# pghysels/STRUMPACK

Measured on AMD Instinct MI355X. Metric: hss_compress_ulv_factor_solve_gflops, higher is better.
Workload: dtype f64

## Files before the change

include/hssk.h:

```cpp
#ifndef HSSK_H
#define HSSK_H

#ifdef __cplusplus
extern "C" {
#endif

typedef struct hssk_ctx hssk_ctx;

int hssk_ctx_create(hssk_ctx** ctx, int device);
void hssk_ctx_destroy(hssk_ctx* ctx);
void* hssk_ctx_stream(hssk_ctx* ctx);
int hssk_sync(hssk_ctx* ctx);
const char* hssk_last_error(void);
typedef struct hssk_plan hssk_plan;
int hssk_plan_begin(hssk_ctx* ctx, hssk_plan** plan);
int hssk_plan_end(hssk_ctx* ctx);
int hssk_plan_replay(hssk_ctx* ctx, hssk_plan* plan);
void hssk_plan_destroy(hssk_plan* plan);
int hssk_plan_size(const hssk_plan* plan);

void* hssk_malloc(long long bytes);
void hssk_free(void* dptr);
long long hssk_device_total_bytes(void);
int hssk_memcpy_h2d(hssk_ctx* ctx, void* dst, const void* src, long long bytes);
int hssk_memcpy_d2h(hssk_ctx* ctx, void* dst, const void* src, long long bytes);
int hssk_upload_async(hssk_ctx* ctx, void* dst, const void* src, long long bytes);
int hssk_memcpy_d2d(hssk_ctx* ctx, void* dst, const void* src, long long bytes);
int hssk_memcpy2d_h2d(hssk_ctx* ctx, void* dst, long long dpitch, const void* src, long long spitch,
                      long long width, long long height);
int hssk_memcpy2d_d2h(hssk_ctx* ctx, void* dst, long long dpitch, const void* src, long long spitch,
                      long long width, long long height);
int hssk_memset_zero(hssk_ctx* ctx, void* dst, long long bytes);
// ... 299 lines not shown
                    double atol, int max_rank, const hssk_elem_src* src, int* res);
int hssk_tree_rcap_max(void);

typedef struct hssk_qr_desc {
  double* A;
  int lda, rows, cols;
  double* Q;
  int ldq, nq;
  double* rdiag;
  double* work;
  int stair;
  double stop_rel, stop_abs;
  int r_only;
} hssk_qr_desc;
int hssk_qr_vbatched(hssk_ctx* ctx, const hssk_qr_desc* descs, int count);
typedef struct hssk_tpqr_desc {
  double* R1;
  int ld1;
  const double* R2;
  int ld2, m;
} hssk_tpqr_desc;
int hssk_tpqr_vbatched(hssk_ctx* ctx, const hssk_tpqr_desc* descs, int count);
int hssk_formq_vbatched(hssk_ctx* ctx, const hssk_qr_desc* descs, int count);

typedef struct hssk_trsm_desc {
  const double* T;
  double* B;
  int n, nrhs, ldt, ldb;
  int lower, transT, unit;
  const double* Tinv;
} hssk_trsm_desc;
int hssk_trsm_vbatched(hssk_ctx* ctx, const hssk_trsm_desc* descs, int count);
typedef struct hssk_lu_desc {
  double* A;
  int n, lda;
  int* piv;
  int* info;
} hssk_lu_desc;
int hssk_getrf_vbatched(hssk_ctx* ctx, const hssk_lu_desc* descs, int count);
typedef struct hssk_lusolve_desc {
  const double* LU;
  const int* piv;
  double* B;
  int n, nrhs, lda, ldb;
} hssk_lusolve_desc;
int hssk_getrs_vbatched(hssk_ctx* ctx, const hssk_lusolve_desc* descs, int count);
// ... 154 lines not shown
```

strumpack_amd/csrc/hip/hssk_rt.h:

```cpp
#pragma once
#include <hip/hip_runtime.h>

#include <cstdio>
#include <stdexcept>
#include <string>

#define HSSK_CHECK(call)                                                                      \
  do {                                                                                        \
    hipError_t e_ = (call);                                                                   \
    if (e_ != hipSuccess)                                                                     \
      throw std::runtime_error(std::string("HIP error: ") + hipGetErrorString(e_) + " at " +  \
                               __FILE__ + ":" + std::to_string(__LINE__));                    \
  } while (0)

namespace hssk_rt {
typedef hipStream_t stream_t;
typedef hipEvent_t event_t;
inline void* dev_malloc(size_t bytes) { void* p = nullptr; if (bytes) HSSK_CHECK(hipMalloc(&p, bytes)); return p; }
inline void dev_free(void* p) { if (p) (void)hipFree(p); }
inline bool pinned_is_device_visible() { return true; }
inline void* pinned_malloc(size_t bytes) { void* p = nullptr; if (bytes) HSSK_CHECK(hipHostMalloc(&p, bytes, hipHostMallocDefault)); return p; }
inline void pinned_free(void* p) { if (p) (void)hipHostFree(p); }
inline void h2d(void* d, const void* h, size_t bytes, stream_t s) { if (bytes) HSSK_CHECK(hipMemcpyAsync(d, h, bytes, hipMemcpyHostToDevice, s)); }
inline void d2h(void* h, const void* d, size_t bytes, stream_t s) { if (bytes) HSSK_CHECK(hipMemcpyAsync(h, d, bytes, hipMemcpyDeviceToHost, s)); }
inline void d2d(void* d, const void* s_, size_t bytes, stream_t s) { if (bytes) HSSK_CHECK(hipMemcpyAsync(d, s_, bytes, hipMemcpyDeviceToDevice, s)); }
inline void h2d_2d(void* d, size_t dpitch, const void* h, size_t hpitch, size_t width, size_t height, stream_t s) {
  if (width && height) HSSK_CHECK(hipMemcpy2DAsync(d, dpitch, h, hpitch, width, height, hipMemcpyHostToDevice, s));
}
inline void d2h_2d(void* h, size_t hpitch, const void* d, size_t dpitch, size_t width, size_t height, stream_t s) {
  if (width && height) HSSK_CHECK(hipMemcpy2DAsync(h, hpitch, d, dpitch, width, height, hipMemcpyDeviceToHost, s));
}
inline void memset_async(void* d, int v, size_t bytes, stream_t s) { if (bytes) HSSK_CHECK(hipMemsetAsync(d, v, bytes, s)); }
inline void sync(stream_t s) { HSSK_CHECK(hipStreamSynchronize(s)); }
inline void check_launch() { HSSK_CHECK(hipGetLastError()); }
template <typename K> inline void allow_dynamic_lds(K kernel, size_t bytes) {
  HSSK_CHECK(hipFuncSetAttribute(reinterpret_cast<const void*>(kernel), hipFuncAttributeMaxDynamicSharedMemorySize, (int)bytes));
}
inline size_t max_lds_per_workgroup() {
  int dev = 0, n = 0;
  if (hipGetDevice(&dev) != hipSuccess) { (void)hipGetLastError(); return 65536; }
  if (hipDeviceGetAttribute(&n, hipDeviceAttributeSharedMemPerBlockOptin, dev) != hipSuccess || n <= 0) {
    (void)hipGetLastError();
    if (hipDeviceGetAttribute(&n, hipDeviceAttributeMaxSharedMemoryPerBlock, dev) != hipSuccess) { (void)hipGetLastError(); return 65536; }
  }
  return n > 0 ? (size_t)n : 65536;
}
inline stream_t stream_create() { stream_t s; HSSK_CHECK(hipStreamCreateWithFlags(&s, hipStreamNonBlocking)); return s; }
inline void stream_destroy(stream_t s) { (void)hipStreamDestroy(s); }
inline event_t event_create() { event_t e; HSSK_CHECK(hipEventCreate(&e)); return e; }
inline void event_destroy(event_t e) { (void)hipEventDestroy(e); }
inline void event_record(event_t e, stream_t s) { HSSK_CHECK(hipEventRecord(e, s)); }
inline float event_elapsed_ms(event_t a, event_t b) { float ms = 0; HSSK_CHECK(hipEventSynchronize(b)); HSSK_CHECK(hipEventElapsedTime(&ms, a, b)); return ms; }
inline void stream_wait_event(stream_t s, event_t e) { HSSK_CHECK(hipStreamWaitEvent(s, e, 0)); }
inline void event_sync(event_t e) { HSSK_CHECK(hipEventSynchronize(e)); }
inline bool is_pinned_host_pointer(const void* p) {
  hipPointerAttribute_t a;
  if (hipPointerGetAttributes(&a, p) != hipSuccess) { (void)hipGetLastError(); return false; }
  return a.type == hipMemoryTypeHost;
}
inline int cu_count() {
  int dev = 0, n = 0;
  if (hipGetDevice(&dev) != hipSuccess || hipDeviceGetAttribute(&n, hipDeviceAttributeMultiprocessorCount, dev) != hipSuccess) { (void)hipGetLastError(); return 256; }
  return n > 0 ? n : 256;
}
inline int coresident_workgroups() { return cu_count(); }
inline size_t device_total_bytes() {
  size_t fr = 0, tot = 0;
  if (hipMemGetInfo(&fr, &tot) != hipSuccess) { (void)hipGetLastError(); return 0; }
  return tot;
}
inline int device_count() { int n = 0; if (hipGetDeviceCount(&n) != hipSuccess) return 0; return n; }
inline void set_device(int d) { HSSK_CHECK(hipSetDevice(d)); }
inline bool is_device_pointer(const void* p) {
  hipPointerAttribute_t a;
  if (hipPointerGetAttributes(&a, p) != hipSuccess) { (void)hipGetLastError(); return false; }
  return a.type == hipMemoryTypeDevice;
}
}
```

strumpack_amd/csrc/host/hss_engine.cpp:

```cpp
#include "hss_engine_internal.hpp"

namespace strumpack {
namespace HSS {

void CommSpec::apply(EngineOptions& e) const {
  e.world = world; e.rank = rank; e.comm_user = user;
  e.allgather = nullptr; e.allgather_stream = nullptr; e.allreduce_stream = nullptr; e.reduce_scatter_stream = nullptr;
  if (world <= 1) return;
  if (native) {
    e.allgather_stream = comm::rccl_allgather_hook;
    e.allreduce_stream = comm::rccl_allreduce_hook;
    e.reduce_scatter_stream = comm::rccl_reduce_scatter_hook;
  } else {
    e.allgather = allgather;
  }
}

DeviceHSS::DeviceHSS(int n, const EngineOptions& opts, const structured::ClusterTree* tree) : n_(n), o_(opts) {
  ck(hssk_ctx_create(&ctx_, o_.device));
  persist_.reset(new Arena(size_t(64) << 20));
  work_.reset(new Arena(size_t(256) << 20));
  fact_.reset(new Arena(size_t(64) << 20));
  tmp_.reset(new Arena(size_t(64) << 20));
  comm_arena_.reset(new Arena(size_t(64) << 20));
  plan_arena_.reset(new Arena(size_t(64) << 20));
  schur_.reset(new Arena(size_t(64) << 20));
  build_tree(tree);
  setup_ownership();
}

DeviceHSS::~DeviceHSS() {
  if (fctx_) hssk_sync(fctx_);
  if (ctx_) hssk_sync(ctx_);
  drop_plans();
  plan_arena_.reset();
  persist_.reset();
  work_.reset();
  fact_.reset();
  tmp_.reset();
  comm_arena_.reset();
  schur_.reset();
  if (fctx_) hssk_ctx_destroy(fctx_);
  hssk_ctx_destroy(ctx_);
}

void DeviceHSS::build_tree(const structured::ClusterTree* tree) {
  nodes_.clear();
  std::function<int(int, int, int, int, const structured::ClusterTree*)> rec =
      [&](int lo, int m, int lvl, int parent, const structured::ClusterTree* t) -> int {
    int id = (int)nodes_.size();
    nodes_.emplace_back();
    nodes_[id].lo = lo; nodes_[id].m = m; nodes_[id].lvl = lvl; nodes_[id].parent = parent;
    bool split = t ? !t->c.empty() : (m > o_.leaf_size);
    if (split) {
      int m0 = t ? t->c[0].size : m / 2;
      int c0 = rec(lo, m0, lvl + 1, id, t ? &t->c[0] : nullptr);
      int c1 = rec(lo + m0, m - m0, lvl + 1, id, t ? &t->c[1] : nullptr);
      nodes_[id].c0 = c0; nodes_[id].c1 = c1;
      nodes_[id].height = 1 + std::max(nodes_[c0].height, nodes_[c1].height);
    }
    return id;
  };
  if (tree && tree->size != n_) throw std::invalid_argument("cluster tree size does not match the matrix dimension");
  rec(0, n_, 0, -1, tree);
  int H = nodes_[0].height, Dp = 0;
// ... 56 lines not shown
```

strumpack_amd/csrc/host/hss_engine.hpp:

```cpp
#pragma once
#include <functional>
#include <iosfwd>
#include <map>
#include <tuple>
#include <memory>
#include <mutex>
#include <string>
#include <vector>

#include "ClusterTree.hpp"
#include "hssk.h"

namespace strumpack {
namespace HSS {

struct EngineOptions {
  double rel_tol = 1e-2, abs_tol = 1e-8;
  int leaf_size = 512, max_rank = 50000, d0 = 128, dd = 64, p = 10;
  int algorithm = 1;
  int random_engine = 0;
  int random_dist = 0;
  int sketch = 0, sjlt_algo = 0, nnz0 = 4, nnz = 4;
  bool user_random = false;
  bool factor_ahead = false;
// ... 247 lines not shown
  std::unique_ptr<Arena> comm_arena_;
  std::unique_ptr<Arena> persist_, work_, fact_, tmp_;
  double *Rt_ = nullptr, *Srt_ = nullptr, *Sct_ = nullptr;
  double *Srt0_ = nullptr, *Sct0_ = nullptr;
  int dcap_ = 0;
  int f32_route_ = 0;
  int attempt_ = 0;
  double* cut_buf_ = nullptr;
  int* cut_idx_ = nullptr;
  size_t cut_buf_cap_ = 0, cut_idx_cap_ = 0;
  int cut_gen_ = -1;
  const int* sj_pat_ = nullptr;
  int sj_nnz_ = 0;
  long long cols_per_rank_ = 0;
  int* d_ranks_ = nullptr;
  struct FactorRun {
    bool active = false, ahead = false, partial = false;
    int sr = 0;
    hssk_ctx* cx = nullptr;
    std::vector<double*> Dh, Vh, Vd;
    std::vector<hssk_trtri_desc> ti;
    std::vector<char> is_cut;
    size_t done = 0;
  } frun_;
  hssk_ctx* fctx_ = nullptr;
  void factor_begin(int sr, bool partial, hssk_ctx* cx);
  void factor_prep(const std::vector<int>& ids);
  void factor_level(const std::vector<int>& ids);
  void factor_ahead_level(size_t h);
  void factor_cancel();
  bool factored_ = false, partial_factored_ = false, schur_ready_ = false;
  void invalidate_factors() { factor_cancel(); factored_ = partial_factored_ = schur_ready_ = false; sub_factored_ = -1; }
  int sub_factored_ = -1;
  std::unique_ptr<Arena> schur_;
  void ensure_dev_tree();
  const hssk_tree_node* dev_tree_ = nullptr;
  int ex_rmax_ = 1, ex_depth_ = 1;
  double *sTheta_ = nullptr, *sPhi_ = nullptr, *sDUB01_ = nullptr, *sVtDUB01_ = nullptr, *sW_ = nullptr;
  PhaseStats stats_;
  std::shared_ptr<HostRng> rng_;
};

}
}
```

strumpack_amd/csrc/host/hss_factor.cpp:

```cpp
#include "hss_engine_internal.hpp"
#include <cstdio>

namespace strumpack {
namespace HSS {

void DeviceHSS::factor() { factor_sub(0, false); }

void DeviceHSS::partial_factor() {
  OpGuard op_guard(op_mu_);
  if (nodes_[0].leaf()) return;
  if (o_.world != 1) throw std::logic_error("partial_factor: needs a single-process matrix");
  factor_sub(nodes_[0].c0, true);
}

void DeviceHSS::factor_begin(int sr, bool partial, hssk_ctx* cx) {
  drop_plans();
  fact_->reset();
  stats_.f_ulv = 0;
  for (auto& nd : nodes_) nd.Qt = nd.Rlq = nd.W1 = nd.Vt0 = nd.Dt = nd.Vt1 = nd.LU = nd.WQ = nd.Tinv = nd.TinvU = nd.Vt0T = nd.Gc = nullptr, nd.piv = nullptr;
  chain_built_ = false;
  if (chain_arena_) chain_arena_->reset();
  const size_t nn = nodes_.size();
  frun_ = FactorRun();
  frun_.active = true;
  frun_.sr = sr; frun_.partial = partial; frun_.cx = cx;
  frun_.Dh.assign(nn, nullptr); frun_.Vh.assign(nn, nullptr); frun_.Vd.assign(nn, nullptr);
  frun_.is_cut.assign(nn, 0);
  if (dist_subtree_) for (int c : cut_nodes_) frun_.is_cut[c] = 1;
}

void DeviceHSS::factor_prep(const std::vector<int>& ids) {
  FactorRun& f = frun_;
  std::vector<hssk_basis_desc> bd;
  for (int id : ids) {
    const Node& nd = nodes_[id];
    if (id == f.sr && !f.partial) continue;
    f.Vh[id] = fact_->dbl((size_t)std::max(nd.mU, 1) * std::max(nd.rV, 1));
    if (!nd.rV) continue;
    double* out = f.Vh[id];
    if (!nd.leaf()) out = f.Vd[id] = fact_->dbl((size_t)nd.mV * nd.rV);
    bd.push_back(hssk_basis_desc{nd.XV, nd.permV, out, nd.mV, nd.rV, nd.rV, nd.mV});
  }
  if (!bd.empty()) ck(hssk_basis_dense(f.cx, bd.data(), (int)bd.size()));
}

void DeviceHSS::factor_level(const std::vector<int>& ids) {
  if (ids.empty()) return;
  FactorRun& f = frun_;
  hssk_ctx* cx = f.cx;
  const int sr = f.sr;
  const bool partial = f.partial;
  std::vector<double*>&Dh = f.Dh, &Vh = f.Vh, &Vd = f.Vd;
  auto dt_slot = [&](int id, int r, int& ld) -> double* {
    const Node& nd = nodes_[id];
    if (nd.parent < 0 || f.is_cut[id]) { ld = std::max(r, 1); return fact_->dbl((size_t)ld * ld); }
    const Node& pa = nodes_[nd.parent];
    const int mu = nodes_[pa.c0].rU + nodes_[pa.c1].rU;
    ld = std::max(mu, 1);
    if (!Dh[nd.parent]) Dh[nd.parent] = fact_->dbl((size_t)ld * ld);
    const int off = id == pa.c0 ? 0 : nodes_[pa.c0].rU;
    return Dh[nd.parent] + off + (size_t)off * ld;
  };
  static const bool no_node = [] { const char* e = std::getenv("STRUMPACK_AMD_NO_ULV_NODE"); return e && e[0] == '1'; }();
  bool fused = !no_node;
  for (int id : ids) {
    const Node& nd = nodes_[id];
// ... 40 lines not shown
      stats_.f_ulv += 2.0 * nd.rV * ((double)a.rU * a.rV + (double)b.rU * b.rV);
    }
  }
  auto node_desc = [&](int id) {
    const Node& nd = nodes_[id];
    const Node &a = nodes_[nd.c0], &b = nodes_[nd.c1];
    hssk_ulvnode_desc d{};
    d.B01 = nd.B01; d.B10 = nd.B10; d.Vt1a = a.Vt1; d.Vt1b = b.Vt1;
    d.ra = a.rU; d.rb = b.rU; d.rva = a.rV; d.rvb = b.rV;
    d.m = a.rU + b.rU;
    d.Dh = Dh[id];
    const bool vh = (id != sr || partial) && nd.rV > 0;
    d.Vd = vh ? Vd[id] : nullptr;
    d.Vh = vh ? Vh[id] : nullptr;
    d.rv = vh ? nd.rV : 0;
    return d;
  };
  if (!cp.empty()) ck(hssk_gather_cols(cx, cp.data(), (int)cp.size()));
  g0.insert(g0.end(), g1.begin(), g1.end());
  if (!g0.empty()) ck(hssk_gemm_vbatched(cx, g0.data(), (int)g0.size()));
  std::vector<hssk_elem_desc> ge;
  std::vector<hssk_ulvsplit_desc> us;
  std::vector<hssk_gemm_desc> g2, g3;
  std::vector<hssk_qr_desc> qr;
  std::vector<hssk_lu_desc> lu;
  for (int id : ids) {
    Node& nd = nodes_[id];
    if (id == sr) {
      const int mu = nd.leaf() ? nd.m : nodes_[nd.c0].rU + nodes_[nd.c1].rU;
      nd.LU = Dh[id];
      if (partial) nd.Vt0 = Vh[id];
      nd.piv = (int*)fact_->alloc(sizeof(int) * (std::max(mu, 1) + 1));
      if (mu) lu.push_back(hssk_lu_desc{nd.LU, mu, mu, nd.piv, nd.piv + mu});
      if (mu && mu <= 256) {
        const size_t nblk = (size_t)(mu + 63) / 64;
        nd.Tinv = fact_->dbl(nblk * 4096);
        nd.TinvU = fact_->dbl(nblk * 4096);
        f.ti.push_back(hssk_trtri_desc{nd.LU, nd.Tinv, mu, mu, 2});
        f.ti.push_back(hssk_trtri_desc{nd.LU, nd.TinvU, mu, mu, 1});
      }
      stats_.f_ulv += 2.0 / 3.0 * mu * (double)mu * mu;
      if (fused) un.push_back(node_desc(id));
      continue;
    }
    const int m = nd.mU, r = nd.rU, rv = nd.rV;
    if (m > r) {
// ... 10 lines not shown
        d.W1 = nd.W1; d.Rlq = nd.Rlq; d.Qt = nd.Qt; d.tau = fact_->dbl((size_t)2 * m);
        d.Vt1 = nd.Vt1; d.Dt = nd.Dt; d.ldt = ldt;
        if (rv) { nd.Vt0T = fact_->dbl((size_t)rv * (m - r)); d.Vt0T = nd.Vt0T; }
        if (r) { nd.WQ = fact_->dbl((size_t)r * (m - r)); d.WQ = nd.WQ; }
        un.push_back(d);
        nd.Tinv = fact_->dbl((size_t)((m - r + 63) / 64) * 4096);
        f.ti.push_back(hssk_trtri_desc{nd.Rlq, nd.Tinv, m - r, m, 0});
        const double k = m - r;
        stats_.f_ulv += 2.0 * k * r * m + (2.0 * m * k * k - 2.0 / 3.0 * k * k * k) + (4.0 * m * m * k - 2.0 * m * k * k) / 1.0 * 0.5 + 2.0 * m * m * rv + 2.0 * r * (double)r * m;
        continue;
      }
      if (m <= 256) {
        us.push_back(hssk_ulvsplit_desc{Dh[id], m, m, r, nd.permU, nd.XU, std::max(r, 1), nd.W1, std::max(r, 1), nd.Rlq, m});
      } else {
        if (r) ge.push_back(hssk_elem_desc{Dh[id], m, nd.permU, nullptr, 0, 0, nd.W1, r, m, r, 0});
        ge.push_back(hssk_elem_desc{Dh[id], m, nd.permU + r, nullptr, 0, 0, nd.Rlq, m - r, m, m, 1});
        if (r) g2.push_back(hssk_gemm_desc{nd.W1, nd.XU, nd.Rlq, m, m - r, r, r, r, m, 1, 0, -1.0, 1.0});
      }
      double* wk = fact_->dbl((size_t)2 * m);
      qr.push_back(hssk_qr_desc{nd.Rlq, m, m, m - r, nd.Qt, m, m, nullptr, wk});
      if (rv) {
        nd.Vt0T = fact_->dbl((size_t)rv * (m - r));
        g3.push_back(hssk_gemm_desc{Vh[id], nd.Qt, nd.Vt0T, rv, m - r, m, m, m, rv, 1, 0, 1.0, 0.0});
        if (r) g3.push_back(hssk_gemm_desc{nd.Qt + (size_t)(m - r) * m, Vh[id], nd.Vt1, r, rv, m, m, m, r, 1, 0, 1.0, 0.0});
      }
      if (r) g3.push_back(hssk_gemm_desc{nd.W1, nd.Qt + (size_t)(m - r) * m, nd.Dt, r, r, m, r, m, ldt, 0, 0, 1.0, 0.0});
      if (r) {
        nd.WQ = fact_->dbl((size_t)r * (m - r));
        g3.push_back(hssk_gemm_desc{nd.W1, nd.Qt, nd.WQ, r, m - r, m, r, m, r, 0, 0, 1.0, 0.0});
      }
      if (m <= 256) {
        nd.Tinv = fact_->dbl((size_t)((m - r + 63) / 64) * 4096);
        f.ti.push_back(hssk_trtri_desc{nd.Rlq, nd.Tinv, m - r, m, 0});
      }
      const double k = m - r;
      stats_.f_ulv += 2.0 * k * r * m + (2.0 * m * k * k - 2.0 / 3.0 * k * k * k) + (4.0 * m * m * k - 2.0 * m * k * k) / 1.0 * 0.5 + 2.0 * m * m * rv + 2.0 * r * (double)r * m;
    } else {
      int ldt = 1;
      nd.Dt = dt_slot(id, m, ldt);
      nd.Vt1 = Vh[id];
      if (m) ge.push_back(hssk_elem_desc{Dh[id], m, nd.permU, nullptr, 0, 0, nd.Dt, m, m, ldt, 0});
    }
  }
  if (!un.empty()) ck(hssk_ulv_node_vbatched(cx, un.data(), (int)un.size()));
  if (!us.empty()) ck(hssk_ulv_split(cx, us.data(), (int)us.size()));
  if (!ge.empty()) ck(hssk_gather_elems(cx, ge.data(), (int)ge.size()));
  if (!g2.empty()) ck(hssk_gemm_vbatched(cx, g2.data(), (int)g2.size()));
  if (!qr.empty()) ck(hssk_qr_vbatched(cx, qr.data(), (int)qr.size()));
  if (!g3.empty()) ck(hssk_gemm_vbatched(cx, g3.data(), (int)g3.size()));
  if (!lu.empty()) ck(hssk_getrf_vbatched(cx, lu.data(), (int)lu.size()));
}

void DeviceHSS::factor_ahead_level(size_t h) {
  if (!o_.factor_ahead || o_.algorithm != 1) return;
  if (o_.world > 1 && !dist_subtree_) return;
  if (!frun_.active) {
    if (h != 0) return;
    if (!fctx_) ck(hssk_ctx_create(&fctx_, o_.device));
    factor_begin(0, false, fctx_);
    frun_.ahead = true;
  }
  if (!frun_.ahead || h >= own_by_height_.size()) return;
  while (frun_.done <= h) {
    const std::vector<int>& ids = own_by_height_[frun_.done];
    for (int id : ids) {
      const Node& nd = nodes_[id];
      if (!nd.compressed()) return;
      if (nd.parent >= 0 && !frun_.is_cut[id]) {
        const Node& pa = nodes_[nd.parent];
        if (!nodes_[pa.c0].compressed() || !nodes_[pa.c1].compressed()) return;
      }
    }
    ck(hssk_stream_wait(fctx_, ctx_));
    factor_prep(ids);
    factor_level(ids);
    if (!frun_.ti.empty()) { ck(hssk_trtri_diag_vbatched(fctx_, frun_.ti.data(), (int)frun_.ti.size())); frun_.ti.clear(); }
    frun_.done++;
  }
}

void DeviceHSS::factor_cancel() {
  if (frun_.active && frun_.ahead && fctx_) hssk_sync(fctx_);
  frun_ = FactorRun();
}

void DeviceHSS::factor_sub(int sr, bool partial) {
  OpGuard op_guard(op_mu_);
  ensure_ready("factor");
  double t0 = now();
  std::vector<std::vector<int>> sub_h;
  if (sr != 0) sub_h = sublists(own_by_height_, sr);
  const std::vector<std::vector<int>>& levels = sr ? sub_h : own_by_height_;
  const bool resume = sr == 0 && !partial && frun_.active && frun_.ahead;
  if (resume) {
    ck(hssk_sync(fctx_));
    ck(hssk_sync(ctx_));
    frun_.cx = ctx_;
  } else {
    static const bool trace_host = [] { const char* e = std::getenv("STRUMPACK_AMD_TRACE_HOST"); return e && e[0] == '1'; }();
    const double th0 = now();
    factor_cancel();
    ck(hssk_sync(ctx_));
    const double th1 = now();
    factor_begin(sr, partial, ctx_);
    const double th2 = now();
// ... 3 lines not shown
      factor_prep(levels[0]);
      const double tp1 = now();
      factor_level(levels[0]);
      frun_.done = 1;
      if (trace_host) std::fprintf(stderr, "# host: factor: prep of the lowest level %.1f us, its launches %.1f us; since the end of compress() %.1f us\n", (tp1 - tp0) * 1e6, (now() - tp1) * 1e6, (tp0 - stats_.t_mark) * 1e6);
    }
    std::vector<int> all;
    for (size_t h = 1; h < levels.size(); h++) all.insert(all.end(), levels[h].begin(), levels[h].end());
    if (dist_subtree_) for (auto& ids : top_by_height_) all.insert(all.end(), ids.begin(), ids.end());
    factor_prep(all);
  }
  for (size_t h = frun_.done; h < levels.size(); h++) {
    if (resume) factor_prep(levels[h]);
    factor_level(levels[h]);
  }
  if (dist_subtree_) {
    exchange_cut_factor();
    for (auto& ids : top_by_height_) {
      if (resume) factor_prep(ids);
      factor_level(ids);
    }
  }
  if (!frun_.ti.empty()) ck(hssk_trtri_diag_vbatched(ctx_, frun_.ti.data(), (int)frun_.ti.size()));
  ck(hssk_sync(ctx_));
  frun_ = FactorRun();
  factored_ = sr == 0;
  sub_factored_ = (sr != 0 && !partial) ? sr : -1;
  partial_factored_ = partial;
  schur_ready_ = false;
  stats_.t_factor = now() - t0;
}

double DeviceHSS::logabsdet() {
  OpGuard op_guard(op_mu_);
  ensure_ready("logabsdet");
  if (o_.world != 1) throw std::logic_error("logabsdet: needs a single-process matrix");
  if (partial_factored_) throw std::logic_error("logabsdet: the factors come from partial_factor() (the (1,1) block is not eliminated)");
  if (!factored_) throw std::logic_error("logabsdet: factor() has not been called (or shift() invalidated the factors)");
  std::vector<hssk_logdet_desc> d;
  for (size_t id = 0; id < nodes_.size(); id++) {
    const Node& nd = nodes_[id];
    if (id == 0) {
      const int mu = nd.leaf() ? nd.m : nodes_[nd.c0].rU + nodes_[nd.c1].rU;
      if (mu) d.push_back(hssk_logdet_desc{nd.LU, mu, mu});
    } else if (nd.mU > nd.rU) {
      d.push_back(hssk_logdet_desc{nd.Rlq, nd.mU - nd.rU, nd.mU});
// ... 16 lines not shown
```

strumpack_amd/csrc/kernels/hssk_ctx.hip:

```cpp
#include "hssk_internal.h"

#include <cstdlib>
#include <unistd.h>

#include <atomic>
#include <condition_variable>
#include <functional>
#include <mutex>
#include <thread>
#include <vector>

static thread_local std::string g_err;
static std::mutex g_pool_mu;
static std::vector<hssk_ctx*> g_pool;
void hssk_set_error(const std::string& msg) { g_err = msg; }

thread_local std::vector<std::function<void()>>* hssk_rec::sink = nullptr;

struct hssk_uploader {
  static constexpr int SLOTS = 4;
  static constexpr size_t CHUNK = size_t(256) << 20;
  hssk_rt::stream_t copy{};
  hssk_rt::event_t ev_copy{}, ev_compute{};
  hssk_rt::event_t ev_mark[2];
// ... 172 lines not shown
int hssk_compute_fence(hssk_ctx* c) {
  HSSK_API_BEGIN
  hssk_uploader* u = uploader(c);
  hssk_rt::event_record(u->ev_compute, c->stream);
  hssk_rt::stream_wait_event(u->copy, u->ev_compute);
  HSSK_API_END
}
int hssk_compute_mark(hssk_ctx* c, int slot) {
  HSSK_API_BEGIN
  hssk_uploader* u = uploader(c);
  hssk_rt::event_record(u->ev_mark[slot & 1], c->stream);
  u->marked[slot & 1] = true;
  HSSK_API_END
}
int hssk_copy_wait(hssk_ctx* c, int slot) {
  HSSK_API_BEGIN
  hssk_uploader* u = uploader(c);
  if (u->marked[slot & 1]) hssk_rt::stream_wait_event(u->copy, u->ev_mark[slot & 1]);
  HSSK_API_END
}

const char* hssk_last_error(void) { return g_err.c_str(); }

int hssk_ctx_create(hssk_ctx** out, int device) {
  HSSK_API_BEGIN
  if (hssk_rt::device_count() <= device)
    throw std::runtime_error("hssk_ctx_create: no HIP device " + std::to_string(device) +
                             " (this library has no CPU fallback)");
  hssk_rt::set_device(device);
  {
    std::lock_guard<std::mutex> g(g_pool_mu);
    for (size_t i = 0; i < g_pool.size(); i++)
      if (g_pool[i]->device == device) {
        *out = g_pool[i];
        g_pool.erase(g_pool.begin() + i);
        return 0;
      }
  }
  hssk_ctx* c = new hssk_ctx;
  c->device = device;
  c->stream = hssk_rt::stream_create();
  c->ring_bytes = size_t(64) << 20;
  c->h_ring = (char*)hssk_rt::pinned_malloc(c->ring_bytes);
  c->zero_copy_bytes = hssk_rt::pinned_is_device_visible() ? 65536 : 0;
  if (const char* e = std::getenv("HSSK_ZERO_COPY_BYTES")) c->zero_copy_bytes = (size_t)std::atoll(e);
  c->d_ring = (char*)hssk_rt::dev_malloc(c->ring_bytes);
  c->ev0 = hssk_rt::event_create();
  c->ev1 = hssk_rt::event_create();
  c->ev_sync = hssk_rt::event_create();
  *out = c;
  HSSK_API_END
}

void hssk_ctx_destroy(hssk_ctx* c) {
  if (!c) return;
  try { hssk_rt::sync(c->stream); } catch (...) {}
  {
    std::lock_guard<std::mutex> g(g_pool_mu);
    if (g_pool.size() < 8) {
      if (c->uploader) c->uploader->release_slots();
      c->ring_off = 0;
      c->dgemm_timed = false;
      if (c->on_side) { c->stream = c->main_saved; c->on_side = false; }
      for (int i = 0; i < 8; i++) {
        for (auto& p : c->watch[i]) { c->watch_free.push_back(p.first); c->watch_free.push_back(p.second); }
        c->watch[i].clear();
        c->watch_open[i] = false;
      }
      c->recording = nullptr;
      c->require_mma = false;
      c->knn_filtered = 0;
      g_pool.push_back(c);
      return;
    }
// ... 268 lines not shown
```

strumpack_amd/csrc/kernels/hssk_internal.h:

```cpp
#pragma once
#include <functional>
#include <vector>
#include <algorithm>
#include <utility>
#include <cstring>
#include <stdexcept>
#include <string>

#include "hssk.h"
#include "hssk_rt.h"

namespace hssk_rec {
extern thread_local std::vector<std::function<void()>>* sink;
}

struct hssk_plan {
  std::vector<std::function<void()>> launches;
  struct Block { char* dev; char* shadow; size_t size; };
  std::vector<Block> blocks;
  size_t off = 0;
  char* alloc(size_t bytes, char** shadow) {
    const size_t need = (bytes + 255) & ~size_t(255);
    if (blocks.empty() || off + need > blocks.back().size) {
      const size_t sz = std::max<size_t>(need, size_t(1) << 20);
      blocks.push_back(Block{(char*)hssk_rt::dev_malloc(sz), (char*)hssk_rt::pinned_malloc(sz), sz});
      off = 0;
    }
    char* p = blocks.back().dev + off;
    *shadow = blocks.back().shadow + off;
    off += need;
    return p;
  }
  ~hssk_plan() { for (auto& b : blocks) { hssk_rt::dev_free(b.dev); hssk_rt::pinned_free(b.shadow); } }
};

struct hssk_uploader;
struct hssk_ctx {
  int device = 0;
  hssk_rt::stream_t stream{};
  char* h_ring = nullptr;
  char* d_ring = nullptr;
  size_t ring_bytes = 0, ring_off = 0;
  size_t zero_copy_bytes = 0;
  hssk_rt::event_t ev0{}, ev1{};
  hssk_rt::event_t ev_sync{};
  hssk_rt::stream_t side{}, main_saved{};
  hssk_rt::event_t ev_fork{}, ev_join{};
  bool on_side = false, side_made = false;
  bool require_mma = false;
  bool dgemm_timed = false;
  double dgemm_timed_flops = 0.;
  struct TimedBracket { hssk_rt::event_t a, b; double flops; };
  std::vector<TimedBracket> dgemm_deferred;
  long long dgemm_trace_wgs = 0;
  long long* d_clk = nullptr;
  double* d_scratch = nullptr;
  struct hssk_uploader* uploader = nullptr;
  int* d_sweep_flags = nullptr;
  int* h_sweep_err = nullptr;
  std::vector<std::pair<hssk_rt::event_t, hssk_rt::event_t>> watch[8];
  std::vector<hssk_rt::event_t> watch_free;
// ... 111 lines not shown
```

strumpack_amd/csrc/kernels/hssk_qr.hip:

```cpp
#include "hssk_backsub.h"
#include "hssk_device.h"
#include "hssk_internal.h"
#include "hssk_qr_reg.h"

#include <algorithm>
#include <cstdlib>
#include <vector>

namespace {

constexpr int QR_THREADS = 512;
constexpr int QR_WAVES = QR_THREADS / 64;

__global__ __launch_bounds__(QR_THREADS) void qr_kernel(const hssk_qr_desc* __restrict__ descs, int qonly) {
  HSSK_SHARED double s_tau;
  const hssk_qr_desc p = descs[blockIdx.x];
  const int tid = threadIdx.x, lane = tid & 63, wave = tid >> 6;
  const int rows = p.rows, cols = p.cols, ld = p.lda;
  double* __restrict__ A = p.A;
  double* taus = p.work;
  const int kmax = rows < cols ? rows : cols;
  double rmax = 0., rmin = 0.;

  for (int k = 0; k < (qonly ? 0 : kmax); k++) {
// ... 150 lines not shown
        hssk_row_sum_n(dot);
#pragma unroll
        for (int c = kc; c < CT; c++) {
          const int col = grp + NC * c;
          if (col > k && col < m) {
            const double tc = st[col];
            const double f = (dot[c] + tc) * tau;
#pragma unroll
            for (int r = 0; r < RC(kc); r++) a[c][r] -= f * vr[r];
            if (l16 == 0) hssk_gstore(R1, (size_t)k + (size_t)col * p.ld1, tc - f);
          }
        }
      }
      if (tid < m) s_t[((k + 1) & 1) * NC * CT + tid] = trow;
    }
  }
}
#undef RC

template <int RT, int CT, int NW>
void launch_qr_reg(hssk_ctx* ctx, const hssk_qr_desc* dd, int count) {
  HSSK_LAUNCH((qr_reg_kernel<RT, CT, NW>), dim3((unsigned)count), dim3(NW * 64), 0, ctx->stream, dd);
}
template <int RT, int CT, int NW>
void launch_formq_reg(hssk_ctx* ctx, const hssk_qr_desc* dd, const hssk_qr_desc* descs, int count) {
  std::vector<QBlock> blocks;
  for (int i = 0; i < count; i++)
    for (int b = 0; b * 4 * NW * CT < descs[i].nq; b++) blocks.push_back(QBlock{i, b});
  if (blocks.empty()) return;
  auto* dw = (const QBlock*)ctx->stage(blocks.data(), sizeof(QBlock) * blocks.size());
  HSSK_LAUNCH((formq_reg_kernel<RT, CT, NW>), dim3((unsigned)blocks.size()), dim3(NW * 64), 0, ctx->stream, dd, dw);
}
void formq_reg(hssk_ctx* ctx, const hssk_qr_desc* dd, const hssk_qr_desc* descs, int count, int rmax) {
  if (rmax <= 64) launch_formq_reg<4, 2, 8>(ctx, dd, descs, count);
  else if (rmax <= 128) launch_formq_reg<8, 4, 8>(ctx, dd, descs, count);
  else if (rmax <= 208) launch_formq_reg<13, 4, 8>(ctx, dd, descs, count);
  else launch_formq_reg<16, 4, 8>(ctx, dd, descs, count);
}

constexpr int QB = 32;
constexpr int QB_MAXROWS = 512;

struct QPanel {
  const double* A;
  const double* tau;
  double* Vc;
  double* VT;
  double* rd_panel;
  double* rdiag;
  int lda, rows, nb, ldv, first;
};

template <int MAXR, int NT>
__global__ __launch_bounds__(NT) void larft_kernel(const QPanel* __restrict__ descs) {
  constexpr int PARTS = NT >= 1024 ? 2 : 1;
  constexpr int LDV = MAXR + 1;
  constexpr int LR = HSSK_BACKSUB_LD;
  HSSK_SHARED double s_V[QB * LDV];
  HSSK_SHARED double s_G[QB * LR];
  HSSK_SHARED double s_rd[64];
// ... 504 lines not shown
    if (!fused) continue;
    for (int i = 0; i < count; i++) {
      const hssk_qr_desc& d = descs[i];
      const int kmax = std::min(d.rows, d.cols);
      if (jg >= kmax || d.nq <= jg) continue;
      WyDesc w{};
      for (int q = std::min(pmax, g0 + GP) - 1; q >= g0; q--) {
        const int jq = q * QB;
        if (jq >= kmax || d.nq <= jq) continue;
        const double* Vq = ws + offV[i] + jq + (size_t)jq * d.rows;
        w.pr[w.np++] = WyPair{Vq + (size_t)d.rows * kmax, Vq, jq - jg, std::min(QB, kmax - jq), d.rows - jq, 0};
      }
      w.C = d.Q + jg + (size_t)jg * d.ldq; w.ldv = d.rows; w.ldc = d.ldq; w.rr = d.rows - jg; w.nc = d.nq - jg;
      wy.push_back(w);
    }
    if (!wy_apply(ctx, wy)) throw std::runtime_error("hssk_qr: fused block reflector refused a block it had accepted");
  }
}

bool force_blocked() {
  static const bool f = [] { const char* e = std::getenv("HSSK_QR_BLOCKED"); return e && e[0] == '1'; }();
  return f;
}

}

extern "C" int hssk_qr_vbatched(hssk_ctx* ctx, const hssk_qr_desc* descs, int count) {
  HSSK_API_BEGIN
  if (count <= 0) return 0;
  int rmax = 0, cmax = 0, qmax = 0;
  for (int i = 0; i < count; i++) {
    rmax = std::max(rmax, descs[i].rows);
    cmax = std::max(cmax, descs[i].cols);
    qmax = std::max(qmax, descs[i].nq);
  }
  static const int blk_rows = [] { const char* e = std::getenv("HSSK_QR_BLOCKED_ROWS"); return e ? std::atoi(e) : 1 << 30; }();
  if (force_blocked() || rmax > 256 || cmax > 224 || (rmax > 208 && cmax > 192) || (rmax >= blk_rows && cmax >= 96 && wy_usable(rmax))) {
    qr_blocked(ctx, descs, count, true);
    hssk_rt::check_launch();
    return 0;
  }
  auto* dd = (const hssk_qr_desc*)ctx->stage(descs, sizeof(*descs) * count);
  if (rmax <= 64 && cmax <= 64) launch_qr_reg<4, 1, 16>(ctx, dd, count);
  else if (rmax <= 128 && cmax <= 128) launch_qr_reg<8, 2, 16>(ctx, dd, count);
  else if (cmax <= 128 && rmax <= 208) launch_qr_reg<13, 4, 8>(ctx, dd, count);
  else if (cmax <= 128) launch_qr_reg<16, 4, 8>(ctx, dd, count);
  else if (rmax > 208) launch_qr_reg<16, 6, 8>(ctx, dd, count);
  else if (cmax <= 160) launch_qr_reg<13, 5, 8>(ctx, dd, count);
  else if (cmax <= 192) launch_qr_reg<13, 6, 8>(ctx, dd, count);
  else launch_qr_reg<13, 7, 8>(ctx, dd, count);
  static const bool q_wy = [] { const char* e = std::getenv("HSSK_QR_FORMQ_WY"); return e && e[0] == '1'; }();
  if (qmax > 0) {
    if (q_wy && rmax >= 128 && cmax >= 64 && wy_usable(rmax)) qr_blocked(ctx, descs, count, false);
    else formq_reg(ctx, dd, descs, count, rmax);
  }
  hssk_rt::check_launch();
  HSSK_API_END
}

extern "C" int hssk_formq_vbatched(hssk_ctx* ctx, const hssk_qr_desc* descs, int count) {
  HSSK_API_BEGIN
  if (count <= 0) return 0;
  int rmax = 0, cmax = 0, qmax = 0;
  for (int i = 0; i < count; i++) {
    rmax = std::max(rmax, descs[i].rows);
    cmax = std::max(cmax, descs[i].cols);
    qmax = std::max(qmax, descs[i].nq);
  }
  if (qmax <= 0) return 0;
  if (force_blocked() || rmax > 256) {
    qr_blocked(ctx, descs, count, false);
  } else {
    static const bool q_wy = [] { const char* e = std::getenv("HSSK_QR_FORMQ_WY"); return e && e[0] == '1'; }();
    if (q_wy && rmax >= 128 && cmax >= 64 && wy_usable(rmax)) qr_blocked(ctx, descs, count, false);
    else {
      auto* dd = (const hssk_qr_desc*)ctx->stage(descs, sizeof(*descs) * count);
      formq_reg(ctx, dd, descs, count, rmax);
    }
  }
  hssk_rt::check_launch();
  HSSK_API_END
}

extern "C" int hssk_tpqr_vbatched(hssk_ctx* ctx, const hssk_tpqr_desc* descs, int count) {
  HSSK_API_BEGIN
  if (count <= 0) return 0;
  int mmax = 0;
  for (int i = 0; i < count; i++) {
    if (descs[i].m < 0 || descs[i].ld1 < descs[i].m || descs[i].ld2 < descs[i].m) HSSK_UNSUPPORTED("bad triangle descriptor");
    mmax = std::max(mmax, descs[i].m);
  }
  if (mmax == 0) return 0;
  if (mmax > 224) HSSK_UNSUPPORTED("triangles beyond 224 columns");
  auto* dd = (const hssk_tpqr_desc*)ctx->stage(descs, sizeof(*descs) * count);
  if (mmax <= 64) HSSK_LAUNCH((tpqr_reg_kernel<4, 2, 8>), dim3((unsigned)count), dim3(512), 0, ctx->stream, dd);
  else if (mmax <= 128) HSSK_LAUNCH((tpqr_reg_kernel<8, 4, 8>), dim3((unsigned)count), dim3(512), 0, ctx->stream, dd);
  else if (mmax <= 208) HSSK_LAUNCH((tpqr_reg_kernel<13, 7, 8>), dim3((unsigned)count), dim3(512), 0, ctx->stream, dd);
  else HSSK_LAUNCH((tpqr_reg_kernel<14, 7, 8>), dim3((unsigned)count), dim3(512), 0, ctx->stream, dd);
  hssk_rt::check_launch();
  HSSK_API_END
}
```

Before: 69910.

## Split leaf ULV factor into critical chain and side-stream work

For leaf-only factor levels, the QR runs without forming Q. Then only the Q column blocks covering the trailing r columns are formed, and only the products that feed the next level run on the main stream. The remaining Q blocks, the off-path GEMMs and the triangular inverses go to a side context on its own stream, joined at factor end, so they overlap with later levels. This adds an extra stream, extra staging and more launches, and optional low-priority or CU-masked stream variants selected by environment variables.

New measurement: 69710 (median of 2 runs). About the same (-0.3%).

```diff
diff --git a/include/hssk.h b/include/hssk.h
--- a/include/hssk.h
+++ b/include/hssk.h
@@ -8,6 +8,7 @@
 typedef struct hssk_ctx hssk_ctx;
 
 int hssk_ctx_create(hssk_ctx** ctx, int device);
+int hssk_ctx_create_side(hssk_ctx** ctx, int device, int kind);
 void hssk_ctx_destroy(hssk_ctx* ctx);
 void* hssk_ctx_stream(hssk_ctx* ctx);
 int hssk_sync(hssk_ctx* ctx);
@@ -353,6 +354,8 @@
 } hssk_tpqr_desc;
 int hssk_tpqr_vbatched(hssk_ctx* ctx, const hssk_tpqr_desc* descs, int count);
 int hssk_formq_vbatched(hssk_ctx* ctx, const hssk_qr_desc* descs, int count);
+int hssk_formq_range_vbatched(hssk_ctx* ctx, const hssk_qr_desc* descs, int count, const int* lo, const int* hi, int outside);
+int hssk_formq_range_supported(const hssk_qr_desc* descs, int count);
 
 typedef struct hssk_trsm_desc {
   const double* T;
diff --git a/strumpack_amd/csrc/hip/hssk_rt.h b/strumpack_amd/csrc/hip/hssk_rt.h
--- a/strumpack_amd/csrc/hip/hssk_rt.h
+++ b/strumpack_amd/csrc/hip/hssk_rt.h
@@ -1,6 +1,7 @@
 #pragma once
 #include <hip/hip_runtime.h>
 
+#include <cstdint>
 #include <cstdio>
 #include <stdexcept>
 #include <string>
@@ -45,7 +46,27 @@
   }
   return n > 0 ? (size_t)n : 65536;
 }
+inline int cu_count_raw() {
+  int dev = 0, n = 0;
+  if (hipGetDevice(&dev) != hipSuccess || hipDeviceGetAttribute(&n, hipDeviceAttributeMultiprocessorCount, dev) != hipSuccess) { (void)hipGetLastError(); return 256; }
+  return n > 0 ? n : 256;
+}
 inline stream_t stream_create() { stream_t s; HSSK_CHECK(hipStreamCreateWithFlags(&s, hipStreamNonBlocking)); return s; }
+inline stream_t stream_create_low_priority() {
+  int least = 0, greatest = 0;
+  HSSK_CHECK(hipDeviceGetStreamPriorityRange(&least, &greatest));
+  stream_t s;
+  HSSK_CHECK(hipStreamCreateWithPriority(&s, hipStreamNonBlocking, least));
+  return s;
+}
+inline stream_t stream_create_off_quarter() {
+  const int words = (cu_count_raw() + 31) / 32;
+  uint32_t mask[32];
+  for (int w = 0; w < 32; w++) mask[w] = 0x77777777u;
+  stream_t s;
+  HSSK_CHECK(hipExtStreamCreateWithCUMask(&s, (uint32_t)(words < 32 ? words : 32), mask));
+  return s;
+}
 inline void stream_destroy(stream_t s) { (void)hipStreamDestroy(s); }
 inline event_t event_create() { event_t e; HSSK_CHECK(hipEventCreate(&e)); return e; }
 inline void event_destroy(event_t e) { (void)hipEventDestroy(e); }
@@ -58,11 +79,7 @@
   if (hipPointerGetAttributes(&a, p) != hipSuccess) { (void)hipGetLastError(); return false; }
   return a.type == hipMemoryTypeHost;
 }
-inline int cu_count() {
-  int dev = 0, n = 0;
-  if (hipGetDevice(&dev) != hipSuccess || hipDeviceGetAttribute(&n, hipDeviceAttributeMultiprocessorCount, dev) != hipSuccess) { (void)hipGetLastError(); return 256; }
-  return n > 0 ? n : 256;
-}
+inline int cu_count() { return cu_count_raw(); }
 inline int coresident_workgroups() { return cu_count(); }
 inline size_t device_total_bytes() {
   size_t fr = 0, tot = 0;
diff --git a/strumpack_amd/csrc/host/hss_engine.cpp b/strumpack_amd/csrc/host/hss_engine.cpp
--- a/strumpack_amd/csrc/host/hss_engine.cpp
+++ b/strumpack_amd/csrc/host/hss_engine.cpp
@@ -31,6 +31,7 @@
 
 DeviceHSS::~DeviceHSS() {
   if (fctx_) hssk_sync(fctx_);
+  if (sctx_) hssk_sync(sctx_);
   if (ctx_) hssk_sync(ctx_);
   drop_plans();
   plan_arena_.reset();
@@ -41,6 +42,7 @@
   comm_arena_.reset();
   schur_.reset();
   if (fctx_) hssk_ctx_destroy(fctx_);
+  if (sctx_) hssk_ctx_destroy(sctx_);
   hssk_ctx_destroy(ctx_);
 }
 
diff --git a/strumpack_amd/csrc/host/hss_engine.hpp b/strumpack_amd/csrc/host/hss_engine.hpp
--- a/strumpack_amd/csrc/host/hss_engine.hpp
+++ b/strumpack_amd/csrc/host/hss_engine.hpp
@@ -293,8 +293,10 @@
     std::vector<hssk_trtri_desc> ti;
     std::vector<char> is_cut;
     size_t done = 0;
+    bool chain_first = false, side = false;
   } frun_;
   hssk_ctx* fctx_ = nullptr;
+  hssk_ctx* sctx_ = nullptr;
   void factor_begin(int sr, bool partial, hssk_ctx* cx);
   void factor_prep(const std::vector<int>& ids);
   void factor_level(const std::vector<int>& ids);
diff --git a/strumpack_amd/csrc/host/hss_factor.cpp b/strumpack_amd/csrc/host/hss_factor.cpp
--- a/strumpack_amd/csrc/host/hss_factor.cpp
+++ b/strumpack_amd/csrc/host/hss_factor.cpp
@@ -1,5 +1,6 @@
 #include "hss_engine_internal.hpp"
 #include <cstdio>
+#include <cstring>
 
 namespace strumpack {
 namespace HSS {
@@ -24,6 +25,8 @@
   frun_ = FactorRun();
   frun_.active = true;
   frun_.sr = sr; frun_.partial = partial; frun_.cx = cx;
+  const char* one = std::getenv("STRUMPACK_AMD_FACTOR_ONE_STREAM");
+  frun_.chain_first = !(one && one[0] == '1');
   frun_.Dh.assign(nn, nullptr); frun_.Vh.assign(nn, nullptr); frun_.Vd.assign(nn, nullptr);
   frun_.is_cut.assign(nn, 0);
   if (dist_subtree_) for (int c : cut_nodes_) frun_.is_cut[c] = 1;
@@ -42,6 +45,13 @@
     bd.push_back(hssk_basis_desc{nd.XV, nd.permV, out, nd.mV, nd.rV, nd.rV, nd.mV});
   }
   if (!bd.empty()) ck(hssk_basis_dense(f.cx, bd.data(), (int)bd.size()));
+}
+
+static int side_stream_kind() {
+  const char* e = std::getenv("STRUMPACK_AMD_FACTOR_SIDE_STREAM");
+  if (e && !std::strcmp(e, "low")) return 1;
+  if (e && !std::strcmp(e, "mask")) return 2;
+  return 0;
 }
 
 void DeviceHSS::factor_level(const std::vector<int>& ids) {
@@ -128,6 +138,9 @@
   std::vector<hssk_elem_desc> ge;
   std::vector<hssk_ulvsplit_desc> us;
   std::vector<hssk_gemm_desc> g2, g3;
+  std::vector<char> g3_side;
+  std::vector<hssk_trtri_desc> ti_s;
+  std::vector<int> q_lo, q_hi;
   std::vector<hssk_qr_desc> qr;
   std::vector<hssk_lu_desc> lu;
   for (int id : ids) {
@@ -184,17 +197,21 @@
       if (rv) {
         nd.Vt0T = fact_->dbl((size_t)rv * (m - r));
         g3.push_back(hssk_gemm_desc{Vh[id], nd.Qt, nd.Vt0T, rv, m - r, m, m, m, rv, 1, 0, 1.0, 0.0});
-        if (r) g3.push_back(hssk_gemm_desc{nd.Qt + (size_t)(m - r) * m, Vh[id], nd.Vt1, r, rv, m, m, m, r, 1, 0, 1.0, 0.0});
-      }
-      if (r) g3.push_back(hssk_gemm_desc{nd.W1, nd.Qt + (size_t)(m - r) * m, nd.Dt, r, r, m, r, m, ldt, 0, 0, 1.0, 0.0});
+        g3_side.push_back(1);
+        if (r) { g3.push_back(hssk_gemm_desc{nd.Qt + (size_t)(m - r) * m, Vh[id], nd.Vt1, r, rv, m, m, m, r, 1, 0, 1.0, 0.0}); g3_side.push_back(0); }
+      }
+      if (r) { g3.push_back(hssk_gemm_desc{nd.W1, nd.Qt + (size_t)(m - r) * m, nd.Dt, r, r, m, r, m, ldt, 0, 0, 1.0, 0.0}); g3_side.push_back(0); }
       if (r) {
         nd.WQ = fact_->dbl((size_t)r * (m - r));
         g3.push_back(hssk_gemm_desc{nd.W1, nd.Qt, nd.WQ, r, m - r, m, r, m, r, 0, 0, 1.0, 0.0});
+        g3_side.push_back(1);
       }
       if (m <= 256) {
         nd.Tinv = fact_->dbl((size_t)((m - r + 63) / 64) * 4096);
-        f.ti.push_back(hssk_trtri_desc{nd.Rlq, nd.Tinv, m - r, m, 0});
-      }
+        ti_s.push_back(hssk_trtri_desc{nd.Rlq, nd.Tinv, m - r, m, 0});
+      }
+      q_lo.push_back(m - r);
+      q_hi.push_back(m);
       const double k = m - r;
       stats_.f_ulv += 2.0 * k * r * m + (2.0 * m * k * k - 2.0 / 3.0 * k * k * k) + (4.0 * m * m * k - 2.0 * m * k * k) / 1.0 * 0.5 + 2.0 * m * m * rv + 2.0 * r * (double)r * m;
     } else {
@@ -208,8 +225,31 @@
   if (!us.empty()) ck(hssk_ulv_split(cx, us.data(), (int)us.size()));
   if (!ge.empty()) ck(hssk_gather_elems(cx, ge.data(), (int)ge.size()));
   if (!g2.empty()) ck(hssk_gemm_vbatched(cx, g2.data(), (int)g2.size()));
-  if (!qr.empty()) ck(hssk_qr_vbatched(cx, qr.data(), (int)qr.size()));
-  if (!g3.empty()) ck(hssk_gemm_vbatched(cx, g3.data(), (int)g3.size()));
+  bool chain_first = f.chain_first && !f.ahead && cx == ctx_ && !qr.empty() && g2.empty();
+  for (int id : ids)
+    if (!nodes_[id].leaf() || id == sr) chain_first = false;
+  if (chain_first && !hssk_formq_range_supported(qr.data(), (int)qr.size())) chain_first = false;
+  if (!chain_first) {
+    if (!qr.empty()) ck(hssk_qr_vbatched(cx, qr.data(), (int)qr.size()));
+    if (!g3.empty()) ck(hssk_gemm_vbatched(cx, g3.data(), (int)g3.size()));
+    f.ti.insert(f.ti.end(), ti_s.begin(), ti_s.end());
+  } else {
+    std::vector<hssk_qr_desc> qr0 = qr;
+    for (auto& d : qr0) d.nq = 0;
+    std::vector<hssk_gemm_desc> gc, gs;
+    for (size_t i = 0; i < g3.size(); i++) (g3_side[i] ? gs : gc).push_back(g3[i]);
+    static const bool trace_host = [] { const char* e = std::getenv("STRUMPACK_AMD_TRACE_HOST"); return e && e[0] == '1'; }();
+    if (trace_host) std::fprintf(stderr, "# host: factor: chain first: %zu leaf panels, %zu + %zu products\n", qr.size(), gc.size(), gs.size());
+    ck(hssk_qr_vbatched(cx, qr0.data(), (int)qr0.size()));
+    ck(hssk_formq_range_vbatched(cx, qr.data(), (int)qr.size(), q_lo.data(), q_hi.data(), 0));
+    if (!gc.empty()) ck(hssk_gemm_vbatched(cx, gc.data(), (int)gc.size()));
+    if (!sctx_) ck(hssk_ctx_create_side(&sctx_, o_.device, side_stream_kind()));
+    f.side = true;
+    ck(hssk_stream_wait(sctx_, cx));
+    ck(hssk_formq_range_vbatched(sctx_, qr.data(), (int)qr.size(), q_lo.data(), q_hi.data(), 1));
+    if (!gs.empty()) ck(hssk_gemm_vbatched(sctx_, gs.data(), (int)gs.size()));
+    if (!ti_s.empty()) ck(hssk_trtri_diag_vbatched(sctx_, ti_s.data(), (int)ti_s.size()));
+  }
   if (!lu.empty()) ck(hssk_getrf_vbatched(cx, lu.data(), (int)lu.size()));
 }
 
@@ -243,6 +283,7 @@
 
 void DeviceHSS::factor_cancel() {
   if (frun_.active && frun_.ahead && fctx_) hssk_sync(fctx_);
+  if (frun_.side && sctx_) hssk_sync(sctx_);
   frun_ = FactorRun();
 }
 
@@ -292,6 +333,7 @@
     }
   }
   if (!frun_.ti.empty()) ck(hssk_trtri_diag_vbatched(ctx_, frun_.ti.data(), (int)frun_.ti.size()));
+  if (frun_.side) ck(hssk_stream_wait(ctx_, sctx_));
   ck(hssk_sync(ctx_));
   frun_ = FactorRun();
   factored_ = sr == 0;
diff --git a/strumpack_amd/csrc/kernels/hssk_ctx.hip b/strumpack_amd/csrc/kernels/hssk_ctx.hip
--- a/strumpack_amd/csrc/kernels/hssk_ctx.hip
+++ b/strumpack_amd/csrc/kernels/hssk_ctx.hip
@@ -1,3 +1,4 @@
+#include "hssk_device.h"
 #include "hssk_internal.h"
 
 #include <cstdlib>
@@ -218,7 +219,14 @@
 
 const char* hssk_last_error(void) { return g_err.c_str(); }
 
-int hssk_ctx_create(hssk_ctx** out, int device) {
+static hssk_rt::stream_t make_stream(int kind) {
+#ifndef HSSK_EMU
+  if (kind == 1) return hssk_rt::stream_create_low_priority();
+  if (kind == 2) return hssk_rt::stream_create_off_quarter();
+#endif
+  return hssk_rt::stream_create();
+}
+static int ctx_create(hssk_ctx** out, int device, int kind) {
   HSSK_API_BEGIN
   if (hssk_rt::device_count() <= device)
     throw std::runtime_error("hssk_ctx_create: no HIP device " + std::to_string(device) +
@@ -227,7 +235,7 @@
   {
     std::lock_guard<std::mutex> g(g_pool_mu);
     for (size_t i = 0; i < g_pool.size(); i++)
-      if (g_pool[i]->device == device) {
+      if (g_pool[i]->device == device && g_pool[i]->kind == kind) {
         *out = g_pool[i];
         g_pool.erase(g_pool.begin() + i);
         return 0;
@@ -235,7 +243,8 @@
   }
   hssk_ctx* c = new hssk_ctx;
   c->device = device;
-  c->stream = hssk_rt::stream_create();
+  c->kind = kind;
+  c->stream = make_stream(kind);
   c->ring_bytes = size_t(64) << 20;
   c->h_ring = (char*)hssk_rt::pinned_malloc(c->ring_bytes);
   c->zero_copy_bytes = hssk_rt::pinned_is_device_visible() ? 65536 : 0;
@@ -246,6 +255,12 @@
   c->ev_sync = hssk_rt::event_create();
   *out = c;
   HSSK_API_END
+}
+
+int hssk_ctx_create(hssk_ctx** out, int device) { return ctx_create(out, device, 0); }
+int hssk_ctx_create_side(hssk_ctx** out, int device, int kind) {
+  if (kind < 0 || kind > 2) { hssk_set_error("hssk_ctx_create_side: kind out of range"); return 1; }
+  return ctx_create(out, device, kind);
 }
 
 void hssk_ctx_destroy(hssk_ctx* c) {
diff --git a/strumpack_amd/csrc/kernels/hssk_internal.h b/strumpack_amd/csrc/kernels/hssk_internal.h
--- a/strumpack_amd/csrc/kernels/hssk_internal.h
+++ b/strumpack_amd/csrc/kernels/hssk_internal.h
@@ -37,6 +37,7 @@
 struct hssk_uploader;
 struct hssk_ctx {
   int device = 0;
+  int kind = 0;
   hssk_rt::stream_t stream{};
   char* h_ring = nullptr;
   char* d_ring = nullptr;
diff --git a/strumpack_amd/csrc/kernels/hssk_qr.hip b/strumpack_amd/csrc/kernels/hssk_qr.hip
--- a/strumpack_amd/csrc/kernels/hssk_qr.hip
+++ b/strumpack_amd/csrc/kernels/hssk_qr.hip
@@ -196,20 +196,32 @@
 void launch_qr_reg(hssk_ctx* ctx, const hssk_qr_desc* dd, int count) {
   HSSK_LAUNCH((qr_reg_kernel<RT, CT, NW>), dim3((unsigned)count), dim3(NW * 64), 0, ctx->stream, dd);
 }
+struct QRange {
+  const int* lo = nullptr;
+  const int* hi = nullptr;
+  bool outside = false;
+};
 template <int RT, int CT, int NW>
-void launch_formq_reg(hssk_ctx* ctx, const hssk_qr_desc* dd, const hssk_qr_desc* descs, int count) {
+void launch_formq_reg(hssk_ctx* ctx, const hssk_qr_desc* dd, const hssk_qr_desc* descs, int count, const QRange& rg) {
+  constexpr int BC = 4 * NW * CT;
   std::vector<QBlock> blocks;
-  for (int i = 0; i < count; i++)
-    for (int b = 0; b * 4 * NW * CT < descs[i].nq; b++) blocks.push_back(QBlock{i, b});
+  for (int i = 0; i < count; i++) {
+    const int nq = descs[i].nq;
+    const int lo = rg.lo ? std::max(rg.lo[i], 0) : 0, hi = rg.lo ? std::min(rg.hi[i], nq) : nq;
+    for (int b = 0; b * BC < nq; b++) {
+      const bool inside = lo < hi && b * BC < hi && lo < (b + 1) * BC;
+      if (inside != rg.outside) blocks.push_back(QBlock{i, b});
+    }
+  }
   if (blocks.empty()) return;
   auto* dw = (const QBlock*)ctx->stage(blocks.data(), sizeof(QBlock) * blocks.size());
   HSSK_LAUNCH((formq_reg_kernel<RT, CT, NW>), dim3((unsigned)blocks.size()), dim3(NW * 64), 0, ctx->stream, dd, dw);
 }
-void formq_reg(hssk_ctx* ctx, const hssk_qr_desc* dd, const hssk_qr_desc* descs, int count, int rmax) {
-  if (rmax <= 64) launch_formq_reg<4, 2, 8>(ctx, dd, descs, count);
-  else if (rmax <= 128) launch_formq_reg<8, 4, 8>(ctx, dd, descs, count);
-  else if (rmax <= 208) launch_formq_reg<13, 4, 8>(ctx, dd, descs, count);
-  else launch_formq_reg<16, 4, 8>(ctx, dd, descs, count);
+void formq_reg(hssk_ctx* ctx, const hssk_qr_desc* dd, const hssk_qr_desc* descs, int count, int rmax, const QRange& rg = QRange()) {
+  if (rmax <= 64) launch_formq_reg<4, 2, 8>(ctx, dd, descs, count, rg);
+  else if (rmax <= 128) launch_formq_reg<8, 4, 8>(ctx, dd, descs, count, rg);
+  else if (rmax <= 208) launch_formq_reg<13, 4, 8>(ctx, dd, descs, count, rg);
+  else launch_formq_reg<16, 4, 8>(ctx, dd, descs, count, rg);
 }
 
 constexpr int QB = 32;
@@ -760,6 +772,14 @@
   static const bool f = [] { const char* e = std::getenv("HSSK_QR_BLOCKED"); return e && e[0] == '1'; }();
   return f;
 }
+bool qr_takes_blocked(int rmax, int cmax) {
+  static const int blk_rows = [] { const char* e = std::getenv("HSSK_QR_BLOCKED_ROWS"); return e ? std::atoi(e) : 1 << 30; }();
+  return force_blocked() || rmax > 256 || cmax > 224 || (rmax > 208 && cmax > 192) || (rmax >= blk_rows && cmax >= 96 && wy_usable(rmax));
+}
+bool formq_takes_wy(int rmax, int cmax) {
+  static const bool q_wy = [] { const char* e = std::getenv("HSSK_QR_FORMQ_WY"); return e && e[0] == '1'; }();
+  return q_wy && rmax >= 128 && cmax >= 64 && wy_usable(rmax);
+}
 
 }
 
@@ -772,8 +792,7 @@
     cmax = std::max(cmax, descs[i].cols);
     qmax = std::max(qmax, descs[i].nq);
   }
-  static const int blk_rows = [] { const char* e = std::getenv("HSSK_QR_BLOCKED_ROWS"); return e ? std::atoi(e) : 1 << 30; }();
-  if (force_blocked() || rmax > 256 || cmax > 224 || (rmax > 208 && cmax > 192) || (rmax >= blk_rows && cmax >= 96 && wy_usable(rmax))) {
+  if (qr_takes_blocked(rmax, cmax)) {
     qr_blocked(ctx, descs, count, true);
     hssk_rt::check_launch();
     return 0;
@@ -787,9 +806,8 @@
   else if (cmax <= 160) launch_qr_reg<13, 5, 8>(ctx, dd, count);
   else if (cmax <= 192) launch_qr_reg<13, 6, 8>(ctx, dd, count);
   else launch_qr_reg<13, 7, 8>(ctx, dd, count);
-  static const bool q_wy = [] { const char* e = std::getenv("HSSK_QR_FORMQ_WY"); return e && e[0] == '1'; }();
   if (qmax > 0) {
-    if (q_wy && rmax >= 128 && cmax >= 64 && wy_usable(rmax)) qr_blocked(ctx, descs, count, false);
+    if (formq_takes_wy(rmax, cmax)) qr_blocked(ctx, descs, count, false);
     else formq_reg(ctx, dd, descs, count, rmax);
   }
   hssk_rt::check_launch();
@@ -809,13 +827,36 @@
   if (force_blocked() || rmax > 256) {
     qr_blocked(ctx, descs, count, false);
   } else {
-    static const bool q_wy = [] { const char* e = std::getenv("HSSK_QR_FORMQ_WY"); return e && e[0] == '1'; }();
-    if (q_wy && rmax >= 128 && cmax >= 64 && wy_usable(rmax)) qr_blocked(ctx, descs, count, false);
+    if (formq_takes_wy(rmax, cmax)) qr_blocked(ctx, descs, count, false);
     else {
       auto* dd = (const hssk_qr_desc*)ctx->stage(descs, sizeof(*descs) * count);
       formq_reg(ctx, dd, descs, count, rmax);
     }
   }
+  hssk_rt::check_launch();
+  HSSK_API_END
+}
+
+extern "C" int hssk_formq_range_supported(const hssk_qr_desc* descs, int count) {
+  int rmax = 0, cmax = 0;
+  for (int i = 0; i < count; i++) {
+    rmax = std::max(rmax, descs[i].rows);
+    cmax = std::max(cmax, descs[i].cols);
+  }
+  return count > 0 && !qr_takes_blocked(rmax, cmax) && !formq_takes_wy(rmax, cmax);
+}
+
+extern "C" int hssk_formq_range_vbatched(hssk_ctx* ctx, const hssk_qr_desc* descs, int count, const int* lo, const int* hi, int outside) {
+  HSSK_API_BEGIN
+  if (count <= 0) return 0;
+  if (!lo || !hi) throw std::invalid_argument("hssk_formq_range_vbatched: null column range");
+  if (!hssk_formq_range_supported(descs, count)) HSSK_UNSUPPORTED("panels outside the register kernels");
+  int rmax = 0;
+  for (int i = 0; i < count; i++) rmax = std::max(rmax, descs[i].rows);
+  auto* dd = (const hssk_qr_desc*)ctx->stage(descs, sizeof(*descs) * count);
+  QRange rg;
+  rg.lo = lo; rg.hi = hi; rg.outside = outside != 0;
+  formq_reg(ctx, dd, descs, count, rmax, rg);
   hssk_rt::check_launch();
   HSSK_API_END
 }
```
